# AILab-CVC/SEED-X

Measured on AMD Instinct MI355X. Metric: end-to-end generations/sec (img-in -> txt + 1024px-img-out), higher is better.
Workload: dtype fp16

## Files before the change

### include/seedx_hip.h

```cpp
#ifndef SEEDX_HIP_H
#define SEEDX_HIP_H
#include <stdint.h>
#ifdef __cplusplus
extern "C" {
#endif

#define SX_OK 0
#define SX_ERR_INVALID 1
#define SX_ERR_HIP 2

#define SX_F16 0
#define SX_BF16 1
#define SX_F32 2
#define SX_BF16X3 3
#define SX_F16X2 4
#define SX_FP8_E4M3 5
#define SX_TILED16 0x100

#define SX_ACT_NONE 0
#define SX_ACT_GELU 1
#define SX_ACT_SILU 2

#define SX_A_LINEAR 0
#define SX_A_CONV3X3 1
// ... 21 lines not shown
  int32_t B, Hin, Win, Cin, Hout, Wout;
  int32_t stride;
  int32_t upsample;
  int32_t ld_bias2d;
  int32_t pad_mode;
  int32_t a_planes;
} sx_gemm_args;
int sx_gemm(const sx_gemm_args* args, void* stream);
int sx_gemm_gn(const sx_gemm_args* args, double* stats, int groups, int rows_per_sample, int* fused_host, void* stream);
typedef struct sx_gemm_ln_args {
  void* x16_out;
  double* row_stats_out;
  const double* row_stats_in;
  const float* colsum;
  int32_t ld_x16;
  int32_t dim;
  float eps;
  int32_t reserved;
} sx_gemm_ln_args;
int sx_gemm_ln(const sx_gemm_args* args, const sx_gemm_ln_args* ln, void* stream);
int sx_gemm_force_tile(int cfg);
int sx_gemm_debug_stamps(void* buf);
int sx_gemm_pick_tile(int M, int N, int K, int glu, int conv);

typedef struct sx_gemv_args {
  const void* x;
  const void* W;
  void* y;
  const float* residual;
  int32_t M, N, K;
  int32_t dtype, out_dtype, act, glu;
  int32_t w_layout;
  int32_t x_layout;
  void* workspace;
  uint64_t workspace_bytes;
  void* x16_out;
  float* row_ssq_out;
  const float* row_ssq_in;
  int32_t ssq_in_parts, ssq_dim;
  float ssq_eps;
  int32_t x_planes;
  int32_t out_planes;
  const float* x16_gamma;
  int32_t w_dtype;
  const float* w_scale;
} sx_gemv_args;
// ... 211 lines not shown
```

### seed-x_amd/_lib.py

```python
import ctypes as C
import os

_HERE = os.path.dirname(os.path.abspath(__file__))
LIB_PATH = os.path.join(_HERE, "lib", "libseedx_hip.so")

SX_F16, SX_BF16, SX_F32 = 0, 1, 2
SX_BF16X3 = 3
SX_F16X2 = 4
SX_FP8_E4M3 = 5
SX_TILED16 = 0x100
SX_ACT_NONE, SX_ACT_GELU, SX_ACT_SILU = 0, 1, 2
SX_A_LINEAR, SX_A_CONV3X3 = 0, 1

c_i32, c_i64, c_f32, c_vp = C.c_int32, C.c_int64, C.c_float, C.c_void_p


class GemmArgs(C.Structure):
    _fields_ = [("A", c_vp), ("W", c_vp), ("C", c_vp), ("bias", c_vp), ("bias2d", c_vp), ("residual", c_vp),
                ("M", c_i32), ("N", c_i32), ("K", c_i32), ("ldc", c_i32), ("ldr", c_i32), ("n_valid", c_i32),
                ("res_mod", c_i32), ("bias2d_rows", c_i32), ("dtype", c_i32), ("out_dtype", c_i32),
                ("act", c_i32), ("glu", c_i32), ("a_mode", c_i32),
                ("B", c_i32), ("Hin", c_i32), ("Win", c_i32), ("Cin", c_i32), ("Hout", c_i32), ("Wout", c_i32),
                ("stride", c_i32), ("upsample", c_i32), ("ld_bias2d", c_i32), ("pad_mode", c_i32), ("a_planes", c_i32)]

# ... 54 lines not shown
                ("v_batch_stride", c_i64), ("v_row_stride", c_i64), ("v_head_stride", c_i64),
                ("o_batch_stride", c_i64), ("o_row_stride", c_i64),
                ("scale", c_f32), ("causal", c_i32), ("dtype", c_i32)]


class AttnSmallArgs(C.Structure):
    _fields_ = [("Q", c_vp), ("K", c_vp), ("V", c_vp), ("O", c_vp),
                ("B", c_i32), ("H", c_i32), ("Sq", c_i32), ("Skv", c_i32), ("D", c_i32),
                ("q_batch_stride", c_i64), ("q_row_stride", c_i64), ("q_head_stride", c_i64),
                ("k_batch_stride", c_i64), ("k_row_stride", c_i64), ("k_head_stride", c_i64),
                ("v_batch_stride", c_i64), ("v_row_stride", c_i64), ("v_head_stride", c_i64),
                ("o_batch_stride", c_i64), ("o_row_stride", c_i64),
                ("scale", c_f32), ("dtype", c_i32)]


SIGNATURES = {
    "sx_version": [],
    "sx_gemm": [C.POINTER(GemmArgs), c_vp],
    "sx_gemm_gn": [C.POINTER(GemmArgs), c_vp, c_i32, c_i32, C.POINTER(c_i32), c_vp],
    "sx_gemm_ln": [C.POINTER(GemmArgs), C.POINTER(GemmLnArgs), c_vp],
    "sx_gemm_force_tile": [c_i32],
    "sx_gemm_debug_stamps": [c_vp],
    "sx_gemm_pick_tile": [c_i32, c_i32, c_i32, c_i32, c_i32],
    "sx_gemv": [C.POINTER(GemvArgs), c_vp],
    "sx_gemv_ssq_parts": [c_i32, c_i32, c_i32],
    "sx_gemv_force_valu": [c_i32],
    "sx_layernorm": [c_vp, c_i32, c_vp, c_i32, c_vp, c_vp, c_i32, c_i32, c_f32, c_i32, c_vp],
    "sx_softmax_rows": [c_vp, c_i64, c_vp, c_i64, c_i32, c_i32, c_f32, c_i32, c_vp],
    "sx_groupnorm": [c_vp, c_vp, c_vp, c_i32, c_vp, c_vp, c_vp, c_i32, c_i32, c_i32, c_i32, c_f32, c_i32, c_vp],
    "sx_groupnorm2": [c_vp, c_vp, c_i32, c_vp, c_vp, c_i32, c_vp, c_vp, c_vp, c_i32, c_i32, c_i32, c_i32, c_f32, c_i32, c_vp],
    "sx_groupnorm_sp": [c_vp, c_vp, c_i32, c_vp, c_vp, c_i32, c_vp, c_vp, c_vp, c_i32, c_i32, c_i32, c_i32, c_i32, c_f32, c_i32,
                        c_i32, c_vp],
    "sx_attention": [C.POINTER(AttnArgs), c_vp],
    "sx_norm_tune": [c_i32, c_i32],
    "sx_gemv_tune": [c_i32, c_i32],
    "sx_comm_alloc": [C.POINTER(c_vp), C.c_uint64],
    "sx_comm_free": [c_vp],
    "sx_ipc_export": [c_vp, C.c_char_p],
    "sx_ipc_open": [C.c_char_p, C.POINTER(c_vp)],
    "sx_ipc_close": [c_vp],
    "sx_allreduce_oneshot": [C.POINTER(OneshotArgs), c_vp],
    "sx_halo_pack": [c_vp, c_vp, c_vp, c_vp, c_i32, c_i32, c_i32, c_i32, c_i32, c_i32, c_vp],
    "sx_attention_small": [C.POINTER(AttnSmallArgs), c_vp],
    "sx_attn_decode": [c_vp, c_vp, c_vp, c_vp, c_vp, c_vp, c_i32, c_i32, c_i32, c_i32, c_f32, c_i32, c_vp],
    "sx_rope_kv_append": [c_vp, c_vp, c_vp, c_vp, c_vp, c_vp, c_i32, c_i32, c_i32, c_i32, c_i32, c_vp],
    "sx_rope_kv_append_b": [c_vp, c_vp, c_vp, c_vp, c_vp, c_vp, c_i32, c_i32, c_i32, c_i32, c_i32, c_i64, c_i32, c_vp],
# ... 66 lines not shown
```

### seed-x_amd/csrc/gemm.hip

```cpp
#include "gemm_common.h"

namespace sxk_gemm {

template <typename TT, int BM, int BN, int WM, int WN, int NSTAGE, int AMODE>
__global__ __launch_bounds__(WM * WN * 64) void gemm_kernel(const GemmP p) {
#if defined(__HIP_DEVICE_COMPILE__)
  typedef typename TT::vec8 vec8;
  constexpr int NW = WM * WN;
  static_assert(NW == 4 || NW == 8, "4 or 8 waves per block");
  constexpr int TM = BM / WM, TN = BN / WN;
  constexpr int FM = TM / 16, FN = TN / 16;
  constexpr bool kGlu = (FN % 2 == 0);
  constexpr int BNP = (BN + 8 * NW - 1) / (8 * NW) * (8 * NW);
  constexpr int A_PER_WAVE = BM / (8 * NW);
  constexpr int B_PER_WAVE = BNP / (8 * NW);
  constexpr int LOADS = A_PER_WAVE + B_PER_WAVE;
  constexpr int A_BYTES = BM * 128, B_BYTES = BNP * 128, STAGE = A_BYTES + B_BYTES;
  static_assert(LOADS * (NSTAGE - 1) <= 63, "vmcnt range");
  extern __shared__ __attribute__((aligned(16))) unsigned char smem[];

  const int tid = threadIdx.x, lane = tid & 63;
  const int wave = __builtin_amdgcn_readfirstlane(tid >> 6);
  const int wm = wave / WN, wn = wave % WN;
  unsigned long long t_start = 0, t_first = 0, t_main = 0;
// ... 309 lines not shown
  if (force >= 0 && force < kNumTiles && (!glu || kTiles[force].glu_ok)) return force;
  int best = 2;
  float best_t = 1e30f;
  for (int c = 0; c < kNumTiles; ++c) {
    const TileCfg& t = kTiles[c];
    if (!((allow >> c) & 1u)) continue;
    if (glu && !t.glu_ok) continue;
    const long tiles = (long)((M + t.bm - 1) / t.bm) * ((N + t.bn - 1) / t.bn);
    const long rounds = (tiles + t.slots - 1) / t.slots;
    const float us = (float)rounds * (conv ? t.a_conv + t.b_conv * (float)K : t.a_lin + t.b_lin * (float)K);
    if (us < best_t) { best_t = us; best = c; }
  }
  return best;
}

}
using namespace sxk_gemm;

static int g_force_tile = -1;
extern "C" int sx_gemm_pick_tile(int M, int N, int K, int glu, int conv) {
  return sxk_gemm::pick_tile(M, N, K, glu != 0, conv != 0, -1, 0x1ff);
}

extern "C" int sx_gemm_debug_stamps(void* buf) {
  sxk_gemm::g_dbg = (unsigned long long*)buf;
  return SX_OK;
}

extern "C" int sx_gemm_force_tile(int cfg) {
  if (cfg == 100 || cfg == 101) { sxk_gemm::g_xcd_2d = cfg - 100; return SX_OK; }
  if (cfg >= 300 && cfg <= 364) { sxk_gemm::g_gm = cfg - 300; return SX_OK; }
  SX_CHECK(cfg >= -1 && cfg < kNumTiles, "sx_gemm_force_tile: %d is not -1, a tile config 0..%d, 100/101 or 300..364", cfg,
           kNumTiles - 1);
  g_force_tile = cfg;
  return SX_OK;
}

static int gemm_impl(const sx_gemm_args* a, double* gn_stats, int gn_groups, int gn_rows, int* gn_fused, const sx_gemm_ln_args* ln,
                     void* stream);

extern "C" int sx_gemm(const sx_gemm_args* a, void* stream) { return gemm_impl(a, nullptr, 0, 0, nullptr, nullptr, stream); }

extern "C" int sx_gemm_ln(const sx_gemm_args* a, const sx_gemm_ln_args* ln, void* stream) {
  SX_CHECK(ln && (ln->row_stats_in || ln->row_stats_out), "sx_gemm_ln: neither a producer nor a consumer role");
  return gemm_impl(a, nullptr, 0, 0, nullptr, ln, stream);
}

extern "C" int sx_gemm_gn(const sx_gemm_args* a, double* stats, int groups, int rows_per_sample, int* fused, void* stream) {
  SX_CHECK(stats && fused && groups > 0 && rows_per_sample > 0, "sx_gemm_gn: bad statistics arguments");
  return gemm_impl(a, stats, groups, rows_per_sample, fused, nullptr, stream);
}

static int gemm_impl(const sx_gemm_args* a, double* gn_stats, int gn_groups, int gn_rows, int* gn_fused, const sx_gemm_ln_args* ln,
                     void* stream) {
  SX_CHECK(a && a->A && a->W && a->C, "sx_gemm: null pointer");
// ... 26 lines not shown
  if (a->a_mode == SX_A_CONV3X3) {
    SX_CHECK(a->Cin % 64 == 0 && a->K == 9 * a->Cin, "sx_gemm conv: Cin=%d K=%d", a->Cin, a->K);
    SX_CHECK(a->stride == 1 || a->stride == 2, "sx_gemm conv: stride");
    SX_CHECK(a->M == a->B * a->Hout * a->Wout, "sx_gemm conv: M != B*Hout*Wout");
    const int hv = a->upsample ? 2 * a->Hin : a->Hin, wv = a->upsample ? 2 * a->Win : a->Win;
    SX_CHECK(a->pad_mode == 0 || a->pad_mode == 1, "sx_gemm conv: pad_mode");
    const int padsum = a->pad_mode ? 1 : 2;
    SX_CHECK(a->Hout == (hv + padsum - 3) / a->stride + 1 && a->Wout == (wv + padsum - 3) / a->stride + 1,
             "sx_gemm conv: output geometry mismatch");
    p.pad = a->pad_mode ? 0 : 1;
    p.Hin = a->Hin; p.Win = a->Win; p.Cin = a->Cin; p.Hout = a->Hout; p.Wout = a->Wout;
    p.stride = a->stride; p.upsample = a->upsample;
    a_bytes = (uint64_t)a->B * a->Hin * a->Win * a->Cin * 2;
  } else {
    SX_CHECK(a->a_mode == SX_A_LINEAR, "sx_gemm: bad a_mode");
    a_bytes = (uint64_t)a->M * Kk * 2;
  }
  const uint64_t w_bytes = (uint64_t)a->N * a->K * 2;
  SX_CHECK(a_bytes < 0x7fffffffull && w_bytes < 0x7fffffffull, "sx_gemm: operand exceeds 2 GiB descriptor range");
  p.a_bytes = (unsigned)a_bytes;
  p.w_bytes = (unsigned)w_bytes;
  hipStream_t st = (hipStream_t)stream;
  p.res_init = (p.residual && p.act == SX_ACT_NONE && !p.glu) ? 1 : 0;
  if (ln) {
    SX_CHECK(a->a_mode == SX_A_LINEAR && !gn_stats, "sx_gemm_ln: linear GEMMs only");
    SX_CHECK(!(ln->row_stats_in && ln->row_stats_out), "sx_gemm_ln: a launch is a producer or a consumer, not both");
    if (ln->row_stats_out) {
      SX_CHECK(ln->x16_out && a->out_dtype == SX_F32 && !a->glu && a->act == SX_ACT_NONE && p.n_valid == a->N,
               "sx_gemm_ln producer: needs x16_out and a plain fp32 output of all N columns");
      SX_CHECK(ln->ld_x16 >= a->N && ln->ld_x16 % 4 == 0 && (((size_t)ln->x16_out) & 7) == 0, "sx_gemm_ln producer: ld_x16=%d", ln->ld_x16);
      p.ln_x16 = ln->x16_out; p.ln_ldx = ln->ld_x16; p.ln_out = ln->row_stats_out;
    } else {
      SX_CHECK(ln->colsum && ln->dim == a->K && ln->eps > 0.f, "sx_gemm_ln consumer: colsum / dim (= K) / eps");
      SX_CHECK(a->out_dtype == a->dtype && !a->residual && !a->bias2d, "sx_gemm_ln consumer: 16-bit output, no residual / bias2d");
      p.ln_in = ln->row_stats_in; p.ln_cs = ln->colsum; p.ln_eps = ln->eps; p.ln_inv_dim = 1.0f / (float)ln->dim;
    }
  }
  unsigned allow = 0x7f;
  if (ln) allow = 0;
  allow |= pp_supported(p, a->dtype, 256, a->a_mode) ? 0x80u : 0u;
  allow |= pp_supported(p, a->dtype, 320, a->a_mode) ? 0x100u : 0u;
  SX_CHECK(!(g_force_tile == 7 || g_force_tile == 8) || ((allow >> g_force_tile) & 1u),
           "sx_gemm: forced ping-pong tile has no kernel for this epilogue");
  if (ln) {
    const int plain = pick_tile(a->M, a->N, Kk, a->glu != 0, false, g_force_tile, 0x1ff);
    SX_CHECK((plain == 7 || plain == 8) && ((allow >> plain) & 1u),
// ... 27 lines not shown
```

### seed-x_amd/csrc/gemm_common.h

```cpp
#pragma once
#include "sx_common.h"

namespace sxk_gemm {

struct GemmP {
  const void* A;
  const void* W;
  void* C;
  const float* bias;
  const float* bias2d;
  const float* residual;
  int M, N, K, ldc, ldr, n_valid, res_mod, bias2d_rows, out_dtype, act, glu;
  int Kw;
  int Hin, Win, Cin, Hout, Wout, stride, upsample, ldb2, pad;
  int tiles_m, tiles_n, xm, xn;
  int gm;
  int res_init;
  unsigned a_bytes, w_bytes;
  unsigned long long* dbg;
  double* gn_stats;
  int gn_cpg, gn_groups, gn_rows;
  void* ln_x16;
  double* ln_out;
  const double* ln_in;
  const float* ln_cs;
  int ln_ldx;
  float ln_eps, ln_inv_dim;
};

template <int N>
__device__ __forceinline__ void wait_vmcnt() {
  asm volatile("s_waitcnt vmcnt(%0)" ::"n"(N) : "memory");
}

__device__ __forceinline__ bool tile_coords(const GemmP& p, int bid, int nblk, int& tile_m, int& tile_n) {
  if (p.xm == 0) {
    const int t = xcd_remap(bid, nblk);
    tile_m = t % p.tiles_m;
    tile_n = t / p.tiles_m;
    return true;
  }
// ... 16 lines not shown
  p.tiles_m = (p.M + BM - 1) / BM;
  p.tiles_n = (p.N + BN - 1) / BN;
  int grid = p.tiles_m * p.tiles_n;
  p.xm = p.xn = 0;
  p.gm = 1;
  if (grid >= 16 && xcd_2d) {
    const double ab = (double)p.M * p.K, wb = (double)p.N * p.K;
    double best = 1e300;
    for (int xm = 1; xm <= 8; xm *= 2) {
      const int xn = 8 / xm;
      if (xm > p.tiles_m || xn > p.tiles_n) continue;
      const long padded = 8L * ((p.tiles_m + xm - 1) / xm) * ((p.tiles_n + xn - 1) / xn);
      const double cost = (ab * xn + wb * xm) * (1.0 + 4.0 * (double)(padded - grid) / grid);
      if (cost < best) { best = cost; p.xm = xm; p.xn = xn; }
    }
    if (p.xm) grid = 8 * ((p.tiles_m + p.xm - 1) / p.xm) * ((p.tiles_n + p.xn - 1) / p.xn);
    p.gm = gm_force > 0 ? gm_force : 8;
  }
  return grid;
}

int launch_pp(const GemmP& p, int dtype, int bn, int a_mode, hipStream_t st);
bool pp_supported(const GemmP& p, int dtype, int bn, int a_mode);

extern unsigned long long* g_dbg;
extern int g_gm;
extern int g_xcd_2d;

}
```

### seed-x_amd/csrc/gemm_pp.hip

```cpp
#include "gemm_common.h"
#include <type_traits>

namespace sxk_gemm {

#define SX_A_CONV3X3_UP 2

#define PP_SYNC()                            \
  do {                                       \
    __builtin_amdgcn_sched_barrier(0);       \
    __builtin_amdgcn_s_barrier();            \
    __builtin_amdgcn_sched_barrier(0);       \
  } while (0)

template <typename TT, int BN, int AMODE, bool OUT32, int ACT, bool GLU, int LN = 0>
__global__ __launch_bounds__(512) void gemm_pp_kernel(const GemmP p) {
#if defined(__HIP_DEVICE_COMPILE__)
  typedef typename TT::vec8 vec8;
  static_assert(LN != 2 || (OUT32 && !GLU && ACT == SX_ACT_NONE), "the LayerNorm producer is the plain fp32-output epilogue");
  constexpr int BM = 256, TN = BN / 4, FN = TN / 16, FM = 8, FH = 4;
  constexpr int NB = BN / 64;
  constexpr int C1 = NB - 3, C2 = 3;
  constexpr int WAITN = 4 + NB;
  constexpr int A_BYTES = BM * 128, STAGE = A_BYTES + BN * 128;
  static_assert(!GLU || FN % 2 == 0, "GLU pairs n-fragments");
  static_assert(BN == 256 || BN == 320, "ping-pong tiles are 256x256 and 256x320");
  extern __shared__ __attribute__((aligned(16))) unsigned char smem[];

  const int tid = threadIdx.x, lane = tid & 63;
  const int wave = __builtin_amdgcn_readfirstlane(tid >> 6);
  const int g = wave >> 2, wc = wave & 3;
  unsigned long long t_start = 0, t_first = 0, t_main = 0;
  if (p.dbg) t_start = __builtin_amdgcn_s_memtime();

  int tile_m, tile_n;
  if (!tile_coords(p, blockIdx.x, gridDim.x, tile_m, tile_n)) return;
  const int m0 = tile_m * BM, n0 = tile_n * BN;

  double ln_s1 = 0.0, ln_s2 = 0.0;
  if constexpr (LN == 1) {
    if (tid < BM) {
      const int m = m0 + tid < p.M ? m0 + tid : p.M - 1;
      ln_s1 = p.ln_in[2 * (size_t)m];
      ln_s2 = p.ln_in[2 * (size_t)m + 1];
    }
  }
  __amdgpu_buffer_rsrc_t rA = __builtin_amdgcn_make_buffer_rsrc((void*)p.A, 0, (int)p.a_bytes, 0x00020000);
// ... 63 lines not shown
        o = a_off[s] + (unsigned)(((t.dy * p.Win + t.dx) * p.Cin + t.cc * 64) * 2);
      }
      voff = ok ? o : 0x80000000u;
    }
    __builtin_amdgcn_raw_ptr_buffer_load_lds(rA, SX_LDS_PTR(smem + buf * STAGE + a_lrow[s] * 128), 16, voff, 0, 0, 0);
  };
  auto dma_w = [&](int i, int buf, int kt) {
    __builtin_amdgcn_raw_ptr_buffer_load_lds(rW, SX_LDS_PTR(smem + buf * STAGE + A_BYTES + (wave * NB + i) * 1024), 16,
                                             w_off[i] + koff_w(kt), 0, 0, 0);
  };
  auto issue_x = [&](int buf, int kt, const Tap& t) {
    dma_a(0, buf, kt, t);
    dma_a(1, buf, kt, t);
#pragma unroll
    for (int i = 0; i < C1; ++i) dma_w(i, buf, kt);
  };
  auto issue_y = [&](int buf, int kt) {
#pragma unroll
    for (int i = C1; i < NB; ++i) dma_w(i, buf, kt);
  };

  f32x4_t acc[FN][FM];
  const int lq = (lane >> 4) * 4;
  if (p.res_init) {
#pragma unroll
    for (int j = 0; j < FM; ++j) {
      const int m = m0 + g * 128 + j * 16 + (lane & 15);
      const int mc = m < p.M ? m : p.M - 1;
      const float* rr = p.residual + (size_t)(p.res_mod ? (mc % p.res_mod) : mc) * p.ldr;
#pragma unroll
      for (int i = 0; i < FN; ++i) {
        int c = n0 + wc * TN + i * 16 + lq;
        if (c + 4 > p.ldr) c = 0;
        acc[i][j] = *(const f32x4_t*)(rr + c);
      }
    }
  } else {
#pragma unroll
    for (int i = 0; i < FN; ++i)
#pragma unroll
      for (int j = 0; j < FM; ++j) acc[i][j] = (f32x4_t){0.f, 0.f, 0.f, 0.f};
  }

  const unsigned frag_row = (unsigned)(lane & 15) * 128u;
  unsigned frag_sw[2];
  frag_sw[0] = (unsigned)(((lane >> 4)) ^ (lane & 7)) << 4;
  frag_sw[1] = (unsigned)((4 + (lane >> 4)) ^ (lane & 7)) << 4;
  const unsigned a_frag = (unsigned)(g * 128) * 128u + frag_row;
  const unsigned w_frag = (unsigned)A_BYTES + (unsigned)(wc * TN) * 128u + frag_row;

  Tap kx = {0, 0, 0}, kz = {0, 0, 0};
  issue_x(0, 0, kx);
  issue_y(0, 0);
  dma_a(2, 0, 0, kz);
  dma_a(3, 0, 0, kz);
  tap_next(kz);
  tap_next(kx);
  issue_x(1, 1, kx);
  issue_y(1, 1);
  tap_next(kx);
  float* ln_lds = (float*)(smem + 2 * STAGE);
  if constexpr (LN == 1) {
    if (tid < BM) {
      const double mu = ln_s1 * (double)p.ln_inv_dim;
      const double var = ln_s2 * (double)p.ln_inv_dim - mu * mu;
      const float rstd = __builtin_amdgcn_rsqf((float)(var > 0.0 ? var : 0.0) + p.ln_eps);
      *(f32x2_t*)(ln_lds + 2 * tid) = (f32x2_t){rstd, -rstd * (float)mu};
    }
  }
  wait_vmcnt<WAITN>();
  PP_SYNC();
  if (p.dbg) t_first = __builtin_amdgcn_s_memtime();
  if (g == 1) PP_SYNC();

  vec8 af[FH], wf0[FN], wf1[FN];

  auto mma = [&](const vec8* wf, int h) {
    __builtin_amdgcn_s_setprio(1);
#pragma unroll
    for (int i = 0; i < FN; ++i)
#pragma unroll
      for (int j = 0; j < FH; ++j) acc[i][h * FH + j] = TT::mfma16(wf[i], af[j], acc[i][h * FH + j]);
    __builtin_amdgcn_s_setprio(0);
  };
  auto lgkm0 = [&]() { asm volatile("s_waitcnt lgkmcnt(0)" ::: "memory"); };

  auto ktile = [&](auto BUFC, int u) {
    constexpr int BUF = decltype(BUFC)::value;
    const unsigned char* sbuf = smem + BUF * STAGE;
#pragma unroll
    for (int j = 0; j < FH; ++j) af[j] = *(const vec8*)(sbuf + a_frag + j * 2048 + frag_sw[0]);
#pragma unroll
    for (int i = 0; i < FN; ++i) wf0[i] = *(const vec8*)(sbuf + w_frag + i * 2048 + frag_sw[0]);
    dma_a(2, BUF ^ 1, u + 1, kz);
    lgkm0();
    PP_SYNC();
    mma(wf0, 0);
    PP_SYNC();
#pragma unroll
    for (int j = 0; j < FH; ++j) af[j] = *(const vec8*)(sbuf + a_frag + j * 2048 + frag_sw[1]);
#pragma unroll
    for (int i = 0; i < FN; ++i) wf1[i] = *(const vec8*)(sbuf + w_frag + i * 2048 + frag_sw[1]);
    dma_a(3, BUF ^ 1, u + 1, kz);
    tap_next(kz);
    wait_vmcnt<WAITN>();
    lgkm0();
    PP_SYNC();
    mma(wf1, 0);
    PP_SYNC();
#pragma unroll
    for (int j = 0; j < FH; ++j) af[j] = *(const vec8*)(sbuf + a_frag + 8192 + j * 2048 + frag_sw[0]);
    issue_x(BUF, u + 2, kx);
    lgkm0();
    PP_SYNC();
    mma(wf0, 1);
    PP_SYNC();
#pragma unroll
    for (int j = 0; j < FH; ++j) af[j] = *(const vec8*)(sbuf + a_frag + 8192 + j * 2048 + frag_sw[1]);
    issue_y(BUF, u + 2);
    tap_next(kx);
    wait_vmcnt<WAITN>();
    lgkm0();
    PP_SYNC();
    mma(wf1, 1);
    PP_SYNC();
  };

  for (int kt = 0; kt < nkt; kt += 2) {
    ktile(std::integral_constant<int, 0>{}, kt);
    if (kt + 1 < nkt) ktile(std::integral_constant<int, 1>{}, kt + 1);
  }
  if (g == 0) PP_SYNC();
  wait_vmcnt<0>();

  if (p.dbg) t_main = __builtin_amdgcn_s_memtime();
  int ncol[FN], nout[FN];
  bool nok[FN];
  f32x4_t bv[FN];
#pragma unroll
  for (int i = 0; i < FN; ++i) {
    const int nb = n0 + wc * TN + i * 16;
    ncol[i] = nb + lq;
    nout[i] = GLU ? (nb >> 1) + lq : ncol[i];
    nok[i] = ncol[i] < p.N && nout[i] < p.n_valid && !(GLU && (i & 1));
    if (ncol[i] >= p.N) ncol[i] = p.N - 4;
    if (nout[i] + 4 > p.ldc) nout[i] = 0;
    bv[i] = (f32x4_t){0.f, 0.f, 0.f, 0.f};
  }
  if (p.bias) {
#pragma unroll
    for (int i = 0; i < FN; ++i) bv[i] = *(const f32x4_t*)(p.bias + ncol[i]);
  }
  const bool b2_uniform = p.bias2d && (m0 / p.bias2d_rows) == ((m0 + BM - 1 < p.M ? m0 + BM - 1 : p.M - 1) / p.bias2d_rows);
  if (b2_uniform) {
    const float* b2 = p.bias2d + (size_t)(m0 / p.bias2d_rows) * p.ldb2;
#pragma unroll
    for (int i = 0; i < FN; ++i) bv[i] += *(const f32x4_t*)(b2 + ncol[i]);
  }
  const bool b2_rows = p.bias2d && !b2_uniform;
  const bool res_late = p.residual && !p.res_init;
  const bool wide = !OUT32 && !GLU && (p.ldc & 7) == 0 && (((size_t)p.C) & 15) == 0;
  bool pair_ok[(FN + 1) / 2];
#pragma unroll
  for (int i = 0; i < (FN + 1) / 2; ++i) {
    const int lim = p.n_valid < p.N ? p.n_valid : p.N;
    pair_ok[i] = (2 * i + 1 < FN) && (n0 + wc * TN + i * 32 + 32 <= lim);
  }
  const bool glu_wide = GLU && !OUT32 && (p.ldc & 7) == 0 && (((size_t)p.C) & 15) == 0 &&
                        ((n0 + wc * TN) >> 1) + 32 <= (p.n_valid < (p.N >> 1) ? p.n_valid : (p.N >> 1));
  auto act1 = [&](f32x4_t x) -> f32x4_t {
    if (ACT == SX_ACT_GELU) {
      const f32x2_t g0 = gelu_erf2((f32x2_t){x[0], x[1]}), g1 = gelu_erf2((f32x2_t){x[2], x[3]});
      return (f32x4_t){g0[0], g0[1], g1[0], g1[1]};
    } else if (ACT == SX_ACT_SILU) {
      return (f32x4_t){silu_f(x[0]), silu_f(x[1]), silu_f(x[2]), silu_f(x[3])};
    }
    return x;
  };
  auto pack4 = [&](f32x4_t x) -> u32x2_t {
    u32x2_t o;
    o[0] = pack2<TT>(x[0], x[1]);
    o[1] = pack2<TT>(x[2], x[3]);
    return o;
  };
  f32x4_t lcs[LN == 1 ? FN : 1];
  if constexpr (LN == 1) {
#pragma unroll
    for (int i = 0; i < FN; ++i) lcs[i] = *(const f32x4_t*)(p.ln_cs + ncol[i]);
  }
  float lsum[LN == 2 ? FM : 1], lsq[LN == 2 ? FM : 1];
  const bool gn = OUT32 && p.gn_stats != nullptr;
  float gsl[FN], gql[FN], gsh[FN], gqh[FN];
#pragma unroll
  for (int i = 0; i < FN; ++i) gsl[i] = gql[i] = gsh[i] = gqh[i] = 0.f;
#pragma unroll
  for (int j = 0; j < FM; ++j) {
    const int m = m0 + g * 128 + j * 16 + (lane & 15);
    const bool mok = m < p.M;
    const int mc = mok ? m : p.M - 1;
    f32x4_t v[FN];
    if constexpr (LN == 1) {
      const f32x2_t ab = *(const f32x2_t*)(ln_lds + 2 * (g * 128 + j * 16 + (lane & 15)));
#pragma unroll
      for (int i = 0; i < FN; ++i) v[i] = acc[i][j] * ab[0] + (lcs[i] * ab[1] + bv[i]);
    } else {
#pragma unroll
      for (int i = 0; i < FN; ++i) v[i] = acc[i][j] + bv[i];
    }
    if (b2_rows) {
      const float* b2 = p.bias2d + (size_t)(mc / p.bias2d_rows) * p.ldb2;
#pragma unroll
      for (int i = 0; i < FN; ++i) v[i] += *(const f32x4_t*)(b2 + ncol[i]);
    }
    if (GLU) {
#pragma unroll
      for (int i = 0; i + 1 < FN; i += 2) {
        const f32x4_t gt = act1(v[i + 1]);
        v[i] = v[i] * gt;
      }
    } else if (ACT != SX_ACT_NONE) {
#pragma unroll
      for (int i = 0; i < FN; ++i) v[i] = act1(v[i]);
    }
    if (res_late) {
      const float* rr = p.residual + (size_t)(p.res_mod ? (mc % p.res_mod) : mc) * p.ldr;
// ... 8 lines not shown
#pragma unroll
      for (int i = 0; i < FN; ++i)
        if (mok && nok[i]) *(f32x4_t*)((float*)p.C + (size_t)m * p.ldc + nout[i]) = v[i];
      if constexpr (LN == 2) {
        float s1 = 0.f, s2 = 0.f;
#pragma unroll
        for (int i = 0; i < FN; ++i) {
          if (mok && nok[i]) {
            s1 += (v[i][0] + v[i][1]) + (v[i][2] + v[i][3]);
            s2 += (v[i][0] * v[i][0] + v[i][1] * v[i][1]) + (v[i][2] * v[i][2] + v[i][3] * v[i][3]);
          }
        }
        lsum[j] = s1;
        lsq[j] = s2;
        const bool xwide = (p.ln_ldx & 7) == 0 && (((size_t)p.ln_x16) & 15) == 0;
#pragma unroll
        for (int i = 0; i < FN; ++i) {
          if ((i & 1) == 0 && i + 1 < FN && xwide && pair_ok[i >> 1]) {
            const u32x2_t o0 = pack4(v[i]), o1 = pack4(v[i + 1]);
            const auto w0 = __builtin_amdgcn_permlane16_swap(o0[0], o1[0], false, false);
            const auto w1 = __builtin_amdgcn_permlane16_swap(o0[1], o1[1], false, false);
            if (mok) {
              const u32x4_t w4 = {w0[0], w1[0], w0[1], w1[1]};
              const int q = lane >> 4;
              const int col = n0 + wc * TN + i * 16 + (q & 1) * 16 + (q >> 1) * 8;
              *(u32x4_t*)((unsigned short*)p.ln_x16 + (size_t)m * p.ln_ldx + col) = w4;
            }
            continue;
          }
          if ((i & 1) && xwide && pair_ok[i >> 1]) continue;
          if (mok && nok[i]) *(u32x2_t*)((unsigned short*)p.ln_x16 + (size_t)m * p.ln_ldx + nout[i]) = pack4(v[i]);
        }
      }
      if (gn && mok) {
#pragma unroll
        for (int i = 0; i < FN; ++i) {
          gsl[i] += v[i][0] + v[i][1];
          gql[i] += v[i][0] * v[i][0] + v[i][1] * v[i][1];
          gsh[i] += v[i][2] + v[i][3];
          gqh[i] += v[i][2] * v[i][2] + v[i][3] * v[i][3];
        }
      }
    } else {
      if constexpr (GLU && FN == 4) {
        if (glu_wide) {
          const u32x2_t o0 = pack4(v[0]), o1 = pack4(v[2]);
          const auto s0 = __builtin_amdgcn_permlane16_swap(o0[0], o1[0], false, false);
          const auto s1 = __builtin_amdgcn_permlane16_swap(o0[1], o1[1], false, false);
          if (mok) {
            const u32x4_t w4 = {s0[0], s1[0], s0[1], s1[1]};
            const int q = lane >> 4;
            const int col = ((n0 + wc * TN) >> 1) + (q & 1) * 16 + (q >> 1) * 8;
            *(u32x4_t*)((unsigned short*)p.C + (size_t)m * p.ldc + col) = w4;
          }
          continue;
        }
      }
#pragma unroll
      for (int i = 0; i < FN; ++i) {
        if (GLU && (i & 1)) continue;
        if (!GLU && wide && (i & 1) == 0 && i + 1 < FN && pair_ok[i >> 1]) {
          const u32x2_t o0 = pack4(v[i]), o1 = pack4(v[i + 1]);
          const auto s0 = __builtin_amdgcn_permlane16_swap(o0[0], o1[0], false, false);
          const auto s1 = __builtin_amdgcn_permlane16_swap(o0[1], o1[1], false, false);
          if (mok) {
            const u32x4_t w4 = {s0[0], s1[0], s0[1], s1[1]};
            const int q = lane >> 4;
            const int col = n0 + wc * TN + i * 16 + (q & 1) * 16 + (q >> 1) * 8;
            *(u32x4_t*)((unsigned short*)p.C + (size_t)m * p.ldc + col) = w4;
          }
          continue;
        }
        if (!GLU && wide && (i & 1) && pair_ok[i >> 1]) continue;
        if (mok && nok[i]) *(u32x2_t*)((unsigned short*)p.C + (size_t)m * p.ldc + nout[i]) = pack4(v[i]);
      }
    }
  }
  if constexpr (LN == 2) {
    float* racc = (float*)smem;
    __syncthreads();
#pragma unroll
    for (int j = 0; j < FM; ++j) {
      float s1 = lsum[j], s2 = lsq[j];
      s1 += __shfl_xor(s1, 16, 64); s2 += __shfl_xor(s2, 16, 64);
      s1 += __shfl_xor(s1, 32, 64); s2 += __shfl_xor(s2, 32, 64);
      if (lane < 16) *(f32x2_t*)(racc + ((size_t)(wc * BM + g * 128 + j * 16 + lane)) * 2) = (f32x2_t){s1, s2};
    }
    __syncthreads();
    if (tid < BM && m0 + tid < p.M) {
      float s1 = 0.f, s2 = 0.f;
#pragma unroll
      for (int w = 0; w < 4; ++w) { s1 += racc[(w * BM + tid) * 2]; s2 += racc[(w * BM + tid) * 2 + 1]; }
      atomicAdd(&p.ln_out[2 * (size_t)(m0 + tid)], (double)s1);
      atomicAdd(&p.ln_out[2 * (size_t)(m0 + tid) + 1], (double)s2);
    }
  }
  if (OUT32 && gn) {
    auto row16_sum = [](float x) -> float {
      x += __builtin_bit_cast(float, __builtin_amdgcn_update_dpp(0, __builtin_bit_cast(int, x), 0xB1, 0xF, 0xF, true));
      x += __builtin_bit_cast(float, __builtin_amdgcn_update_dpp(0, __builtin_bit_cast(int, x), 0x4E, 0xF, 0xF, true));
      x += __builtin_bit_cast(float, __builtin_amdgcn_update_dpp(0, __builtin_bit_cast(int, x), 0x141, 0xF, 0xF, true));
      x += __builtin_bit_cast(float, __builtin_amdgcn_update_dpp(0, __builtin_bit_cast(int, x), 0x140, 0xF, 0xF, true));
      return x;
    };
#pragma unroll
    for (int i = 0; i < FN; ++i) {
      gsl[i] = row16_sum(gsl[i]);
      gql[i] = row16_sum(gql[i]);
      gsh[i] = row16_sum(gsh[i]);
      gqh[i] = row16_sum(gqh[i]);
    }
    float* gslot = (float*)smem;
    const int gbase = n0 / p.gn_cpg;
    const int nlast = (n0 + BN < p.N ? n0 + BN : p.N) - 1;
    const int ngr = nlast / p.gn_cpg - gbase + 1;
    __syncthreads();
    if ((lane & 15) == 0) {
#pragma unroll
      for (int i = 0; i < FN; ++i) {
        const int cp = (wc * TN + i * 16 + lq) >> 1;
        *(f32x4_t*)(gslot + ((size_t)g * (BN / 2) + cp) * 2) = (f32x4_t){gsl[i], gql[i], gsh[i], gqh[i]};
      }
    }
    __syncthreads();
    const int smp = m0 / p.gn_rows;
    for (int t = tid; t < 2 * ngr; t += 512) {
      const int G = gbase + (t >> 1), which = t & 1;
      int c_lo = G * p.gn_cpg - n0, c_hi = (G + 1) * p.gn_cpg - n0;
      c_lo = c_lo < 0 ? 0 : c_lo;
      const int c_end = (p.N - n0 < BN ? p.N - n0 : BN);
      c_hi = c_hi > c_end ? c_end : c_hi;
      float acc = 0.f;
      for (int cp = c_lo >> 1; cp < (c_hi >> 1); ++cp) acc += gslot[(size_t)cp * 2 + which];
      for (int cp = c_lo >> 1; cp < (c_hi >> 1); ++cp) acc += gslot[((size_t)(BN / 2) + cp) * 2 + which];
      atomicAdd(&p.gn_stats[((size_t)smp * p.gn_groups + G) * 2 + which], (double)acc);
    }
  }
  if (p.dbg) {
    asm volatile("s_waitcnt vmcnt(0)" ::: "memory");
    const unsigned long long t_end = __builtin_amdgcn_s_memtime();
    if (tid == 0) {
      unsigned long long* d = p.dbg + (size_t)blockIdx.x * 4;
      d[0] = t_start; d[1] = t_first; d[2] = t_main; d[3] = t_end;
    }
  }
#endif
}

template <typename TT, int BN, int AMODE, bool OUT32, int ACT, bool GLU, int LN = 0>
static int launch_one(const GemmP& p0, hipStream_t st) {
  GemmP p = p0;
  p.dbg = g_dbg;
  const int grid = plan_grid(p, 256, BN, g_xcd_2d, g_gm);
  constexpr size_t lds = 2 * (size_t)(256 + BN) * 128 + (LN == 1 ? 2048 : 0);
  auto k = gemm_pp_kernel<TT, BN, AMODE, OUT32, ACT, GLU, LN>;
  static hipError_t attr[16];
  static bool done[16];
  int dev = 0;
  (void)hipGetDevice(&dev);
  dev &= 15;
  if (!done[dev]) {
    attr[dev] = hipFuncSetAttribute((const void*)k, hipFuncAttributeMaxDynamicSharedMemorySize, (int)lds);
    done[dev] = true;
  }
  SX_CHECK(attr[dev] == hipSuccess, "sx_gemm: cannot reserve %zu B of LDS for the 256x%d ping-pong tile: %s", lds, BN,
           hipGetErrorString(attr[dev]));
  hipLaunchKernelGGL(k, dim3(grid), dim3(512), lds, st, p);
  SX_HIP_LAUNCH_CHECK();
  return SX_OK;
}

static int epi_code(const GemmP& p, int dtype) {
  const bool out32 = p.out_dtype == SX_F32;
  if (!out32 && p.out_dtype != dtype) return -1;
  if (p.glu) {
    if (out32) return -1;
    if (p.act == SX_ACT_GELU) return 2;
    if (p.act == SX_ACT_SILU) return 3;
    return -1;
  }
  if (p.act == SX_ACT_NONE) return out32 ? 4 : 0;
  if (p.act == SX_ACT_GELU && !out32) return 1;
  return -1;
}

bool pp_supported(const GemmP& p, int dtype, int bn, int a_mode) {
  const int e = epi_code(p, dtype);
  if (e < 0) return false;
  if (p.ln_in && !(a_mode == SX_A_LINEAR && (e == 0 || e == 2) && !p.ln_out)) return false;
  if (p.ln_out && !(a_mode == SX_A_LINEAR && e == 4 && !p.gn_stats)) return false;
  if (bn == 320 && (e == 2 || e == 3)) return false;
  if (a_mode == SX_A_CONV3X3 && !(e == 0 || e == 4)) return false;
  if (a_mode == SX_A_CONV3X3 && p.upsample && !(p.stride == 1 && p.pad == 1)) return false;
  return bn == 256 || bn == 320;
}

template <typename TT>
static int launch_t(const GemmP& p, int dtype, int bn, int a_mode, hipStream_t st) {
  const int e = epi_code(p, dtype);
#define PP_CASE(BNV, AM, O32, ACTV, GLUV) return launch_one<TT, BNV, AM, O32, ACTV, GLUV>(p, st)
  if (p.ln_in) {
    if (e == 2) return launch_one<TT, 256, SX_A_LINEAR, false, SX_ACT_GELU, true, 1>(p, st);
    if (bn == 256) return launch_one<TT, 256, SX_A_LINEAR, false, SX_ACT_NONE, false, 1>(p, st);
    return launch_one<TT, 320, SX_A_LINEAR, false, SX_ACT_NONE, false, 1>(p, st);
  }
  if (p.ln_out) {
    if (bn == 256) return launch_one<TT, 256, SX_A_LINEAR, true, SX_ACT_NONE, false, 2>(p, st);
    return launch_one<TT, 320, SX_A_LINEAR, true, SX_ACT_NONE, false, 2>(p, st);
  }
  if (a_mode == SX_A_LINEAR) {
    if (bn == 256) {
      switch (e) {
        case 0: PP_CASE(256, SX_A_LINEAR, false, SX_ACT_NONE, false);
        case 1: PP_CASE(256, SX_A_LINEAR, false, SX_ACT_GELU, false);
        case 2: PP_CASE(256, SX_A_LINEAR, false, SX_ACT_GELU, true);
        case 3: PP_CASE(256, SX_A_LINEAR, false, SX_ACT_SILU, true);
        case 4: PP_CASE(256, SX_A_LINEAR, true, SX_ACT_NONE, false);
      }
    } else {
// ... 14 lines not shown
        case 0: PP_CASE(320, SX_A_CONV3X3, false, SX_ACT_NONE, false);
        case 4: PP_CASE(320, SX_A_CONV3X3, true, SX_ACT_NONE, false);
      }
    }
  } else {
    if (bn == 256) {
      switch (e) {
        case 0: PP_CASE(256, SX_A_CONV3X3_UP, false, SX_ACT_NONE, false);
        case 4: PP_CASE(256, SX_A_CONV3X3_UP, true, SX_ACT_NONE, false);
      }
    } else {
      switch (e) {
        case 0: PP_CASE(320, SX_A_CONV3X3_UP, false, SX_ACT_NONE, false);
        case 4: PP_CASE(320, SX_A_CONV3X3_UP, true, SX_ACT_NONE, false);
      }
    }
  }
#undef PP_CASE
  return -1;
}

int launch_pp(const GemmP& p, int dtype, int bn, int a_mode, hipStream_t st) {
  if (!pp_supported(p, dtype, bn, a_mode)) return -1;
  return dtype == SX_BF16 ? launch_t<BF16>(p, dtype, bn, a_mode, st) : launch_t<F16>(p, dtype, bn, a_mode, st);
}

}
```

Before: 1.304.

## Stream residual fragments into accumulators during early K-steps of ping-pong GEMM

For ping-pong GEMMs with an fp32 residual-init epilogue, some accumulator fragments now start at zero. Their residual values are fetched by buffer-to-LDS DMA during the first NST K-tiles and added into the accumulators there. This hides the up-front residual load latency behind MFMA work. In exchange it costs extra LDS, more template instantiations and inline-asm MFMAs, and adds vmcnt accounting plus a lane-ID recompute in the epilogue.

```diff
diff --git a/include/seedx_hip.h b/include/seedx_hip.h
--- a/include/seedx_hip.h
+++ b/include/seedx_hip.h
@@ -67,6 +67,7 @@
 int sx_gemm_force_tile(int cfg);
 int sx_gemm_debug_stamps(void* buf);
 int sx_gemm_pick_tile(int M, int N, int K, int glu, int conv);
+int sx_gemm_residual_stream(int tile, int K);
 
 typedef struct sx_gemv_args {
   const void* x;
diff --git a/seed-x_amd/_lib.py b/seed-x_amd/_lib.py
--- a/seed-x_amd/_lib.py
+++ b/seed-x_amd/_lib.py
@@ -100,6 +100,7 @@
     "sx_gemm_force_tile": [c_i32],
     "sx_gemm_debug_stamps": [c_vp],
     "sx_gemm_pick_tile": [c_i32, c_i32, c_i32, c_i32, c_i32],
+    "sx_gemm_residual_stream": [c_i32, c_i32],
     "sx_gemv": [C.POINTER(GemvArgs), c_vp],
     "sx_gemv_ssq_parts": [c_i32, c_i32, c_i32],
     "sx_gemv_force_valu": [c_i32],
diff --git a/seed-x_amd/csrc/gemm.hip b/seed-x_amd/csrc/gemm.hip
--- a/seed-x_amd/csrc/gemm.hip
+++ b/seed-x_amd/csrc/gemm.hip
@@ -355,6 +355,11 @@
   return sxk_gemm::pick_tile(M, N, K, glu != 0, conv != 0, -1, 0x1ff);
 }
 
+extern "C" int sx_gemm_residual_stream(int tile, int K) {
+  if ((tile != 7 && tile != 8) || K <= 0 || K % 64) return -1;
+  return sxk_gemm::pp_rs_fragments(tile == 7 ? 256 : 320, K);
+}
+
 extern "C" int sx_gemm_debug_stamps(void* buf) {
   sxk_gemm::g_dbg = (unsigned long long*)buf;
   return SX_OK;
@@ -363,7 +368,9 @@
 extern "C" int sx_gemm_force_tile(int cfg) {
   if (cfg == 100 || cfg == 101) { sxk_gemm::g_xcd_2d = cfg - 100; return SX_OK; }
   if (cfg >= 300 && cfg <= 364) { sxk_gemm::g_gm = cfg - 300; return SX_OK; }
-  SX_CHECK(cfg >= -1 && cfg < kNumTiles, "sx_gemm_force_tile: %d is not -1, a tile config 0..%d, 100/101 or 300..364", cfg,
+  if (cfg == 601 || cfg == 602) { sxk_gemm::g_rs_mode = cfg == 601 ? -1 : 0; return SX_OK; }
+  if (cfg >= 611 && cfg <= 613) { sxk_gemm::g_rs_mode = cfg - 610; return SX_OK; }
+  SX_CHECK(cfg >= -1 && cfg < kNumTiles, "sx_gemm_force_tile: %d is not -1, a tile config 0..%d, 100/101, 300..364, 601/602 or 611..613", cfg,
            kNumTiles - 1);
   g_force_tile = cfg;
   return SX_OK;
@@ -436,6 +443,10 @@
   p.w_bytes = (unsigned)w_bytes;
   hipStream_t st = (hipStream_t)stream;
   p.res_init = (p.residual && p.act == SX_ACT_NONE && !p.glu) ? 1 : 0;
+  if (p.residual) {
+    const uint64_t r_bytes = ((uint64_t)((a->res_mod ? a->res_mod : a->M) - 1) * a->ldr + (a->ldr < n_out ? a->ldr : n_out)) * 4;
+    p.r_bytes = r_bytes < 0x7fffffffull ? (unsigned)r_bytes : 0u;
+  }
   if (ln) {
     SX_CHECK(a->a_mode == SX_A_LINEAR && !gn_stats, "sx_gemm_ln: linear GEMMs only");
     SX_CHECK(!(ln->row_stats_in && ln->row_stats_out), "sx_gemm_ln: a launch is a producer or a consumer, not both");
diff --git a/seed-x_amd/csrc/gemm_common.h b/seed-x_amd/csrc/gemm_common.h
--- a/seed-x_amd/csrc/gemm_common.h
+++ b/seed-x_amd/csrc/gemm_common.h
@@ -17,6 +17,7 @@
   int gm;
   int res_init;
   unsigned a_bytes, w_bytes;
+  unsigned r_bytes;
   unsigned long long* dbg;
   double* gn_stats;
   int gn_cpg, gn_groups, gn_rows;
@@ -79,9 +80,11 @@
 
 int launch_pp(const GemmP& p, int dtype, int bn, int a_mode, hipStream_t st);
 bool pp_supported(const GemmP& p, int dtype, int bn, int a_mode);
+int pp_rs_fragments(int bn, int K);
 
 extern unsigned long long* g_dbg;
 extern int g_gm;
 extern int g_xcd_2d;
+extern int g_rs_mode;
 
 }
diff --git a/seed-x_amd/csrc/gemm_pp.hip b/seed-x_amd/csrc/gemm_pp.hip
--- a/seed-x_amd/csrc/gemm_pp.hip
+++ b/seed-x_amd/csrc/gemm_pp.hip
@@ -3,7 +3,20 @@
 
 namespace sxk_gemm {
 
+#define PP_RS_256_L1 8
+#define PP_RS_256_L2 16
+#define PP_RS_320_L1 8
+#define PP_RS_320_L2 18
+#define PP_RS_320_L3 40
+#define PP_RS_256_K1 10
+#define PP_RS_256_K2 20
+#define PP_RS_320_K1 10
+#define PP_RS_320_K2 20
+#define PP_RS_320_K3 64
+
 #define SX_A_CONV3X3_UP 2
+
+constexpr int pp_rs_rpk(int bn) { return bn == 256 ? 2 : 1; }
 
 #define PP_SYNC()                            \
   do {                                       \
@@ -12,7 +25,15 @@
     __builtin_amdgcn_sched_barrier(0);       \
   } while (0)
 
-template <typename TT, int BN, int AMODE, bool OUT32, int ACT, bool GLU, int LN = 0>
+template <int B, int E, class F>
+__device__ __forceinline__ void static_for(F&& f) {
+  if constexpr (B < E) {
+    f(std::integral_constant<int, B>{});
+    static_for<B + 1, E>(f);
+  }
+}
+
+template <typename TT, int BN, int AMODE, bool OUT32, int ACT, bool GLU, int LN = 0, int NST = 0>
 __global__ __launch_bounds__(512) void gemm_pp_kernel(const GemmP p) {
 #if defined(__HIP_DEVICE_COMPILE__)
   typedef typename TT::vec8 vec8;
@@ -22,6 +43,11 @@
   constexpr int C1 = NB - 3, C2 = 3;
   constexpr int WAITN = 4 + NB;
   constexpr int A_BYTES = BM * 128, STAGE = A_BYTES + BN * 128;
+  constexpr bool RS = NST > 0;
+  constexpr int NF = FM * FN, RPK = pp_rs_rpk(BN), RS_S = NST * RPK;
+  constexpr int RS_BASE = 2 * STAGE, RS_WSTR = 2 * RPK * 1024;
+  static_assert(!RS || (OUT32 && ACT == SX_ACT_NONE && !GLU && AMODE == SX_A_LINEAR && LN != 1), "residual streaming: plain fp32 epilogue, linear A");
+  static_assert(RS_S <= NF && FN % RPK == 0, "streamed fragments; the fragments of one step share a row block");
   static_assert(!GLU || FN % 2 == 0, "GLU pairs n-fragments");
   static_assert(BN == 256 || BN == 320, "ping-pong tiles are 256x256 and 256x320");
   extern __shared__ __attribute__((aligned(16))) unsigned char smem[];
@@ -131,17 +157,46 @@
 
   f32x4_t acc[FN][FM];
   const int lq = (lane >> 4) * 4;
-  if (p.res_init) {
+  __amdgpu_buffer_rsrc_t rR = __builtin_amdgcn_make_buffer_rsrc((void*)p.residual, 0, RS ? (int)p.r_bytes : 0, 0x00020000);
+  if constexpr (RS) {
 #pragma unroll
     for (int j = 0; j < FM; ++j) {
-      const int m = m0 + g * 128 + j * 16 + (lane & 15);
-      const int mc = m < p.M ? m : p.M - 1;
-      const float* rr = p.residual + (size_t)(p.res_mod ? (mc % p.res_mod) : mc) * p.ldr;
+      if (j * FN + FN > RS_S) {
+        const int m = m0 + g * 128 + j * 16 + (lane & 15);
+        const unsigned ro = (unsigned)(p.res_mod ? m % p.res_mod : m) * (unsigned)p.ldr * 4u + (unsigned)(n0 + wc * TN + lq) * 4u;
+#pragma unroll
+        for (int i = 0; i < FN; ++i)
+          if (j * FN + i >= RS_S) acc[i][j] = __builtin_bit_cast(f32x4_t, __builtin_amdgcn_raw_buffer_load_b128(rR, ro + i * 64, 0, 0));
+      }
 #pragma unroll
       for (int i = 0; i < FN; ++i) {
-        int c = n0 + wc * TN + i * 16 + lq;
-        if (c + 4 > p.ldr) c = 0;
-        acc[i][j] = *(const f32x4_t*)(rr + c);
+        if (j * FN + i < RS_S) {
+          acc[i][j] = (f32x4_t){0.f, 0.f, 0.f, 0.f};
+          asm volatile("" : "+v"(acc[i][j]));
+        }
+      }
+    }
+  } else if (RS || p.res_init) {
+#pragma unroll
+    for (int j = 0; j < FM; ++j) {
+      if (j * FN + FN > RS_S) {
+        const int m = m0 + g * 128 + j * 16 + (lane & 15);
+        const int mc = m < p.M ? m : p.M - 1;
+        const float* rr = p.residual + (size_t)(p.res_mod ? (mc % p.res_mod) : mc) * p.ldr;
+#pragma unroll
+        for (int i = 0; i < FN; ++i) {
+          if (j * FN + i < RS_S) continue;
+          int c = n0 + wc * TN + i * 16 + lq;
+          if (c + 4 > p.ldr) c = 0;
+          acc[i][j] = *(const f32x4_t*)(rr + c);
+        }
+      }
+#pragma unroll
+      for (int i = 0; i < FN; ++i) {
+        if (j * FN + i < RS_S) {
+          acc[i][j] = (f32x4_t){0.f, 0.f, 0.f, 0.f};
+          asm volatile("" : "+v"(acc[i][j]));
+        }
       }
     }
   } else {
@@ -158,6 +213,30 @@
   const unsigned a_frag = (unsigned)(g * 128) * 128u + frag_row;
   const unsigned w_frag = (unsigned)A_BYTES + (unsigned)(wc * TN) * 128u + frag_row;
 
+  const unsigned rs_cb = (unsigned)(n0 + wc * TN + lq) * 4u;
+  unsigned rs_rb = 0;
+  unsigned rs_d16 = 0, rs_lim = 0xffffffffu;
+  if constexpr (RS) {
+    const int row0 = m0 + g * 128 + (lane & 15);
+    const unsigned rowb = (unsigned)p.ldr * 4u;
+    rs_rb = (unsigned)(p.res_mod ? row0 % p.res_mod : row0) * rowb;
+    rs_d16 = (unsigned)(p.res_mod ? 16 % p.res_mod : 16) * rowb;
+    if (p.res_mod) rs_lim = (unsigned)p.res_mod * rowb;
+  }
+  unsigned char* rs_lds = smem + RS_BASE + wave * RS_WSTR;
+  auto rs_issue = [&](auto SC) {
+    constexpr int s = decltype(SC)::value;
+    constexpr int j = (s * RPK) / FN, i0 = (s * RPK) % FN;
+    if constexpr (s > 0 && i0 == 0) {
+      rs_rb += rs_d16;
+      if (rs_rb >= rs_lim) rs_rb -= rs_lim;
+    }
+    (void)j;
+    static_assert(RPK <= 2, "one DMA per fragment of a step (the instruction offset is a literal)");
+    __builtin_amdgcn_raw_ptr_buffer_load_lds(rR, SX_LDS_PTR(rs_lds + (s & 1) * RPK * 1024), 16, rs_rb + rs_cb, 0, i0 * 64, 0);
+    if constexpr (RPK == 2)
+      __builtin_amdgcn_raw_ptr_buffer_load_lds(rR, SX_LDS_PTR(rs_lds + ((s & 1) * RPK + 1) * 1024), 16, rs_rb + rs_cb, 0, (i0 + 1) * 64, 0);
+  };
   Tap kx = {0, 0, 0}, kz = {0, 0, 0};
   issue_x(0, 0, kx);
   issue_y(0, 0);
@@ -189,13 +268,25 @@
 #pragma unroll
     for (int i = 0; i < FN; ++i)
 #pragma unroll
-      for (int j = 0; j < FH; ++j) acc[i][h * FH + j] = TT::mfma16(wf[i], af[j], acc[i][h * FH + j]);
+      for (int j = 0; j < FH; ++j) {
+        if constexpr (RS) {
+          if (std::is_same<TT, BF16>::value)
+            asm volatile("v_mfma_f32_16x16x32_bf16 %0, %1, %2, %0" : "+v"(acc[i][h * FH + j]) : "v"(wf[i]), "v"(af[j]));
+          else
+            asm volatile("v_mfma_f32_16x16x32_f16 %0, %1, %2, %0" : "+v"(acc[i][h * FH + j]) : "v"(wf[i]), "v"(af[j]));
+        } else {
+          acc[i][h * FH + j] = TT::mfma16(wf[i], af[j], acc[i][h * FH + j]);
+        }
+      }
     __builtin_amdgcn_s_setprio(0);
   };
   auto lgkm0 = [&]() { asm volatile("s_waitcnt lgkmcnt(0)" ::: "memory"); };
 
-  auto ktile = [&](auto BUFC, int u) {
+  auto ktile = [&](auto BUFC, auto STC, int u) {
     constexpr int BUF = decltype(BUFC)::value;
+    constexpr int ST = decltype(STC)::value;
+    constexpr bool rs_iss = RS && ST >= 0 && ST < NST;
+    constexpr bool rs_add = RS && ST >= 1 && ST - 1 < NST;
     const unsigned char* sbuf = smem + BUF * STAGE;
 #pragma unroll
     for (int j = 0; j < FH; ++j) af[j] = *(const vec8*)(sbuf + a_frag + j * 2048 + frag_sw[0]);
@@ -212,8 +303,9 @@
     for (int i = 0; i < FN; ++i) wf1[i] = *(const vec8*)(sbuf + w_frag + i * 2048 + frag_sw[1]);
     dma_a(3, BUF ^ 1, u + 1, kz);
     tap_next(kz);
-    wait_vmcnt<WAITN>();
+    wait_vmcnt<WAITN + (rs_add ? RPK : 0)>();
     lgkm0();
+    if constexpr (rs_iss) rs_issue(std::integral_constant<int, (ST >= 0 ? ST : 0)>{});
     PP_SYNC();
     mma(wf1, 0);
     PP_SYNC();
@@ -228,29 +320,58 @@
     for (int j = 0; j < FH; ++j) af[j] = *(const vec8*)(sbuf + a_frag + 8192 + j * 2048 + frag_sw[1]);
     issue_y(BUF, u + 2);
     tap_next(kx);
-    wait_vmcnt<WAITN>();
-    lgkm0();
+    wait_vmcnt<WAITN + (rs_iss ? RPK : 0)>();
+    if constexpr (rs_add) {
+      constexpr int s = ST - 1, j = (s * RPK) / FN, i0 = (s * RPK) % FN;
+      f32x4_t rf[RPK];
+#pragma unroll
+      for (int r = 0; r < RPK; ++r) rf[r] = *(const f32x4_t*)(rs_lds + ((s & 1) * RPK + r) * 1024 + lane * 16);
+      lgkm0();
+#pragma unroll
+      for (int r = 0; r < RPK; ++r) acc[i0 + r][j] += rf[r];
+      if constexpr (RPK == 2) asm volatile("s_nop 1" : "+v"(acc[i0][j]), "+v"(acc[i0 + 1][j]));
+      else asm volatile("s_nop 1" : "+v"(acc[i0][j]));
+    } else {
+      lgkm0();
+    }
     PP_SYNC();
     mma(wf1, 1);
     PP_SYNC();
   };
 
-  for (int kt = 0; kt < nkt; kt += 2) {
-    ktile(std::integral_constant<int, 0>{}, kt);
-    if (kt + 1 < nkt) ktile(std::integral_constant<int, 1>{}, kt + 1);
+  constexpr int KT0 = RS ? NST + 1 : 0;
+  if constexpr (RS) {
+    int ku = 0;
+    static_for<0, KT0>([&](auto U) {
+      constexpr int u = decltype(U)::value;
+      asm volatile("" : "+s"(ku));
+      ktile(std::integral_constant<int, (u & 1)>{}, std::integral_constant<int, u>{}, ku);
+      ++ku;
+    });
+    if constexpr (KT0 & 1) {
+      if (KT0 < nkt) ktile(std::integral_constant<int, 1>{}, std::integral_constant<int, -1>{}, KT0);
+    }
+  }
+  for (int kt = KT0 + (KT0 & 1); kt < nkt; kt += 2) {
+    ktile(std::integral_constant<int, 0>{}, std::integral_constant<int, -1>{}, kt);
+    if (kt + 1 < nkt) ktile(std::integral_constant<int, 1>{}, std::integral_constant<int, -1>{}, kt + 1);
   }
   if (g == 0) PP_SYNC();
   wait_vmcnt<0>();
+  if constexpr (RS) asm volatile("s_nop 7\n\ts_nop 7" ::: "memory");
 
   if (p.dbg) t_main = __builtin_amdgcn_s_memtime();
+  int lane_e = lane;
+  if constexpr (RS) lane_e = (int)__builtin_amdgcn_mbcnt_hi(~0u, __builtin_amdgcn_mbcnt_lo(~0u, 0u));
+  const int lq_e = RS ? (lane_e >> 4) * 4 : lq;
   int ncol[FN], nout[FN];
   bool nok[FN];
   f32x4_t bv[FN];
 #pragma unroll
   for (int i = 0; i < FN; ++i) {
     const int nb = n0 + wc * TN + i * 16;
-    ncol[i] = nb + lq;
-    nout[i] = GLU ? (nb >> 1) + lq : ncol[i];
+    ncol[i] = nb + lq_e;
+    nout[i] = GLU ? (nb >> 1) + lq_e : ncol[i];
     nok[i] = ncol[i] < p.N && nout[i] < p.n_valid && !(GLU && (i & 1));
     if (ncol[i] >= p.N) ncol[i] = p.N - 4;
     if (nout[i] + 4 > p.ldc) nout[i] = 0;
@@ -267,7 +388,7 @@
     for (int i = 0; i < FN; ++i) bv[i] += *(const f32x4_t*)(b2 + ncol[i]);
   }
   const bool b2_rows = p.bias2d && !b2_uniform;
-  const bool res_late = p.residual && !p.res_init;
+  const bool res_late = !RS && p.residual && !p.res_init;
   const bool wide = !OUT32 && !GLU && (p.ldc & 7) == 0 && (((size_t)p.C) & 15) == 0;
   bool pair_ok[(FN + 1) / 2];
 #pragma unroll
@@ -304,12 +425,12 @@
   for (int i = 0; i < FN; ++i) gsl[i] = gql[i] = gsh[i] = gqh[i] = 0.f;
 #pragma unroll
   for (int j = 0; j < FM; ++j) {
-    const int m = m0 + g * 128 + j * 16 + (lane & 15);
+    const int m = m0 + g * 128 + j * 16 + (lane_e & 15);
     const bool mok = m < p.M;
     const int mc = mok ? m : p.M - 1;
     f32x4_t v[FN];
     if constexpr (LN == 1) {
-      const f32x2_t ab = *(const f32x2_t*)(ln_lds + 2 * (g * 128 + j * 16 + (lane & 15)));
+      const f32x2_t ab = *(const f32x2_t*)(ln_lds + 2 * (g * 128 + j * 16 + (lane_e & 15)));
 #pragma unroll
       for (int i = 0; i < FN; ++i) v[i] = acc[i][j] * ab[0] + (lcs[i] * ab[1] + bv[i]);
     } else {
@@ -364,7 +485,7 @@
             const auto w1 = __builtin_amdgcn_permlane16_swap(o0[1], o1[1], false, false);
             if (mok) {
               const u32x4_t w4 = {w0[0], w1[0], w0[1], w1[1]};
-              const int q = lane >> 4;
+              const int q = lane_e >> 4;
               const int col = n0 + wc * TN + i * 16 + (q & 1) * 16 + (q >> 1) * 8;
               *(u32x4_t*)((unsigned short*)p.ln_x16 + (size_t)m * p.ln_ldx + col) = w4;
             }
@@ -391,7 +512,7 @@
           const auto s1 = __builtin_amdgcn_permlane16_swap(o0[1], o1[1], false, false);
           if (mok) {
             const u32x4_t w4 = {s0[0], s1[0], s0[1], s1[1]};
-            const int q = lane >> 4;
+            const int q = lane_e >> 4;
             const int col = ((n0 + wc * TN) >> 1) + (q & 1) * 16 + (q >> 1) * 8;
             *(u32x4_t*)((unsigned short*)p.C + (size_t)m * p.ldc + col) = w4;
           }
@@ -407,7 +528,7 @@
           const auto s1 = __builtin_amdgcn_permlane16_swap(o0[1], o1[1], false, false);
           if (mok) {
             const u32x4_t w4 = {s0[0], s1[0], s0[1], s1[1]};
-            const int q = lane >> 4;
+            const int q = lane_e >> 4;
             const int col = n0 + wc * TN + i * 16 + (q & 1) * 16 + (q >> 1) * 8;
             *(u32x4_t*)((unsigned short*)p.C + (size_t)m * p.ldc + col) = w4;
           }
@@ -426,7 +547,7 @@
       float s1 = lsum[j], s2 = lsq[j];
       s1 += __shfl_xor(s1, 16, 64); s2 += __shfl_xor(s2, 16, 64);
       s1 += __shfl_xor(s1, 32, 64); s2 += __shfl_xor(s2, 32, 64);
-      if (lane < 16) *(f32x2_t*)(racc + ((size_t)(wc * BM + g * 128 + j * 16 + lane)) * 2) = (f32x2_t){s1, s2};
+      if (lane_e < 16) *(f32x2_t*)(racc + ((size_t)(wc * BM + g * 128 + j * 16 + lane_e)) * 2) = (f32x2_t){s1, s2};
     }
     __syncthreads();
     if (tid < BM && m0 + tid < p.M) {
@@ -457,10 +578,10 @@
     const int nlast = (n0 + BN < p.N ? n0 + BN : p.N) - 1;
     const int ngr = nlast / p.gn_cpg - gbase + 1;
     __syncthreads();
-    if ((lane & 15) == 0) {
+    if ((lane_e & 15) == 0) {
 #pragma unroll
       for (int i = 0; i < FN; ++i) {
-        const int cp = (wc * TN + i * 16 + lq) >> 1;
+        const int cp = (wc * TN + i * 16 + lq_e) >> 1;
         *(f32x4_t*)(gslot + ((size_t)g * (BN / 2) + cp) * 2) = (f32x4_t){gsl[i], gql[i], gsh[i], gqh[i]};
       }
     }
@@ -489,13 +610,14 @@
 #endif
 }
 
-template <typename TT, int BN, int AMODE, bool OUT32, int ACT, bool GLU, int LN = 0>
+template <typename TT, int BN, int AMODE, bool OUT32, int ACT, bool GLU, int LN = 0, int NST = 0>
 static int launch_one(const GemmP& p0, hipStream_t st) {
   GemmP p = p0;
   p.dbg = g_dbg;
   const int grid = plan_grid(p, 256, BN, g_xcd_2d, g_gm);
-  constexpr size_t lds = 2 * (size_t)(256 + BN) * 128 + (LN == 1 ? 2048 : 0);
-  auto k = gemm_pp_kernel<TT, BN, AMODE, OUT32, ACT, GLU, LN>;
+  constexpr size_t lds = 2 * (size_t)(256 + BN) * 128 + (LN == 1 ? 2048 : 0) + (NST > 0 ? 8 * 2 * pp_rs_rpk(BN) * 1024 : 0);
+  static_assert(lds <= 160 * 1024, "LDS of a CU");
+  auto k = gemm_pp_kernel<TT, BN, AMODE, OUT32, ACT, GLU, LN, NST>;
   static hipError_t attr[16];
   static bool done[16];
   int dev = 0;
@@ -537,6 +659,52 @@
   return bn == 256 || bn == 320;
 }
 
+int g_rs_mode = -1;
+static const int kRsSteps[2][3] = {{PP_RS_256_L1, PP_RS_256_L2, PP_RS_256_L2}, {PP_RS_320_L1, PP_RS_320_L2, PP_RS_320_L3}};
+
+int pp_rs_steps(const GemmP& p, int dtype, int bn, int a_mode) {
+  if (g_rs_mode < 0 || a_mode != SX_A_LINEAR || !p.residual || !p.res_init || p.ln_in || p.out_dtype != SX_F32 || p.r_bytes == 0) return 0;
+  const int nkt = p.K / 64;
+  const int* menu = kRsSteps[bn == 320];
+  int lvl;
+  if (g_rs_mode > 0) {
+    lvl = g_rs_mode;
+  } else {
+    lvl = bn == 320 ? (nkt >= PP_RS_320_K3 ? 3 : nkt >= PP_RS_320_K2 ? 2 : nkt >= PP_RS_320_K1 ? 1 : 0)
+                    : (nkt >= PP_RS_256_K2 ? 2 : nkt >= PP_RS_256_K1 ? 1 : 0);
+  }
+  int nst = 0;
+  for (int l = 0; l < lvl && l < 3; ++l)
+    if (nkt > menu[l]) nst = menu[l];
+  return nst;
+}
+
+int pp_rs_fragments(int bn, int K) {
+  GemmP p;
+  memset(&p, 0, sizeof(p));
+  p.K = K; p.residual = (const float*)&p; p.res_init = 1; p.out_dtype = SX_F32; p.r_bytes = 4;
+  return pp_rs_steps(p, SX_F16, bn, SX_A_LINEAR) * pp_rs_rpk(bn);
+}
+
+template <typename TT, int BN, int NST>
+static int launch_rs_one(const GemmP& p, hipStream_t st) {
+  if (p.ln_out) return launch_one<TT, BN, SX_A_LINEAR, true, SX_ACT_NONE, false, 2, NST>(p, st);
+  return launch_one<TT, BN, SX_A_LINEAR, true, SX_ACT_NONE, false, 0, NST>(p, st);
+}
+
+template <typename TT>
+static int launch_rs(const GemmP& p, int bn, int nst, hipStream_t st) {
+  if (bn == 256) {
+    if (nst == PP_RS_256_L1) return launch_rs_one<TT, 256, PP_RS_256_L1>(p, st);
+    if (nst == PP_RS_256_L2) return launch_rs_one<TT, 256, PP_RS_256_L2>(p, st);
+  } else {
+    if (nst == PP_RS_320_L1) return launch_rs_one<TT, 320, PP_RS_320_L1>(p, st);
+    if (nst == PP_RS_320_L2) return launch_rs_one<TT, 320, PP_RS_320_L2>(p, st);
+    if (nst == PP_RS_320_L3) return launch_rs_one<TT, 320, PP_RS_320_L3>(p, st);
+  }
+  return -1;
+}
+
 template <typename TT>
 static int launch_t(const GemmP& p, int dtype, int bn, int a_mode, hipStream_t st) {
   const int e = epi_code(p, dtype);
@@ -597,6 +765,8 @@
 
 int launch_pp(const GemmP& p, int dtype, int bn, int a_mode, hipStream_t st) {
   if (!pp_supported(p, dtype, bn, a_mode)) return -1;
+  if (const int nst = pp_rs_steps(p, dtype, bn, a_mode))
+    return dtype == SX_BF16 ? launch_rs<BF16>(p, bn, nst, st) : launch_rs<F16>(p, bn, nst, st);
   return dtype == SX_BF16 ? launch_t<BF16>(p, dtype, bn, a_mode, st) : launch_t<F16>(p, dtype, bn, a_mode, st);
 }
 
```

After: 1.304 (median of 2 runs). No clear change (+0.0%).
